# NVlabs/ODISE

Hardware: NVIDIA H100
Metric: images/sec @1024x1024 panoptic inference (ODISE hot path) (higher is better)
Workload: dtype f16q8

## Files before the change

include/odise_b200.h:

```cpp
#ifndef ODISE_B200_H_
#define ODISE_B200_H_

#include <stdint.h>

#ifdef __cplusplus
extern "C" {
#endif

#define ODISE_OK 0
#define ODISE_ERR_ARG 10001
#define ODISE_ERR_ALIGN 10002
#define ODISE_ERR_DRIVER 10003
#define ODISE_ERR_TENSORMAP 10004
#define ODISE_ERR_WORKSPACE 10005
#define ODISE_ERR_UNSUPPORTED 10006

#define ODISE_ACT_NONE 0
#define ODISE_ACT_RELU 1
#define ODISE_ACT_SILU 2
#define ODISE_ACT_GELU 3
#define ODISE_ACT_QUICKGELU 4

#define ODISE_PLANES_BF16 0
#define ODISE_PLANES_F16 1
// ... 96 lines not shown
int odise_msda_fused_box_backward_det_f16(const void* value, const int64_t* spatial_shapes, const int64_t* level_start,
                                          const float* ref, const void* offs, const void* logits, const void* grad_out,
                                          void* grad_value, void* grad_offs, void* grad_logits,
                                          int N, int S, int M, int D, int L, int Lq, int P, void* workspace,
                                          void* stream);
int odise_msda_fused_box_backward_det_bf16(const void* value, const int64_t* spatial_shapes,
                                           const int64_t* level_start, const float* ref, const void* offs,
                                           const void* logits, const void* grad_out, void* grad_value,
                                           void* grad_offs, void* grad_logits, int N, int S, int M, int D, int L,
                                           int Lq, int P, void* workspace, void* stream);

typedef struct odise_gemm_desc {
  int M, N, K, batch;
  int nmma;
  int conv3x3;
  int conv_C, conv_H, conv_W;
  const void* a_hi; const void* a_lo; long long lda; long long a_batch_stride;
  const void* b_hi; const void* b_lo; long long ldb; long long b_batch_stride;
  float alpha;
  const float* bias;
  const float* rowbias; int rows_per_group; long long rowbias_ld;
  int act;
  const float* residual; long long ld_residual; long long residual_batch_stride;
  float* out_f32; long long ld_out; long long out_batch_stride;
  void* out_hi; void* out_lo; long long ld_out_bf16; long long out_bf16_batch_stride;
  int split_k; void* workspace; long long workspace_bytes;
  int force_bn;
  const float* bias_m;
  int conv_mode;
  int geglu;
  float* gn_partial;
  long long gn_seg_stride; long long gn_plane_stride;
  int out_planes_fp16;
} odise_gemm_desc;
int odise_gemm_bf16(const odise_gemm_desc* desc, void* stream);
int odise_gemm_tile_policy(int M, int N, int K, int batch, int conv3x3, int nmma, int* bn, int* pair);
int odise_profile_begin(void);
int odise_profile_end(long long* launches, double* total_ms, double* total_flops);


int odise_split_f32(const float* x, long long ldx, void* hi, void* lo, long long ldo, long long rows, int cols,
                    void* stream);
int odise_split_f16_f32(const float* x, long long ldx, void* hi, void* lo, long long ldo, long long rows, int cols,
                        void* stream);
int odise_groupnorm_stats_f32(const float* x, long long ldx, float* mean, float* rstd, int B, int HW, int C, int G,
                              float eps, void* stream);
int odise_groupnorm_stats_bs_f32(const float* x, long long ldx, long long x_bs, float* mean, float* rstd, int B,
                                 int HW, int C, int G, float eps, void* stream);
long long odise_groupnorm_ws_floats(int B, int HW, int C, int G);
int odise_groupnorm_stats_ws_f32(const float* x, long long ldx, long long x_bs, float* ws, float* mean, float* rstd,
                                 int B, int HW, int C, int G, float eps, void* stream);
int odise_groupnorm_finalize_seg_f32(const float* partial, long long seg_stride, long long plane_stride, float* mean,
                                     float* rstd, int B, int HW, int C, int G, float eps, void* stream);
int odise_groupnorm_apply_f32(const float* x, long long ldx, const float* mean, const float* rstd,
                              const float* gamma, const float* beta, int act, float* y, long long ldy, void* hi,
                              void* lo, long long ldo, int B, int HW, int C, int G, void* stream);
int odise_groupnorm_apply_bs_f32(const float* x, long long ldx, long long x_bs, const float* mean, const float* rstd,
                                 const float* gamma, const float* beta, int act, float* y, long long ldy,
                                 long long y_bs, void* hi, void* lo, long long ldo, long long o_bs, int B, int HW,
                                 int C, int G, void* stream);
int odise_groupnorm_apply_res_f32(const float* x, long long ldx, const float* mean, const float* rstd,
                                  const float* gamma, const float* beta, const float* res, long long ldres, int act,
                                  float* y, long long ldy, int accumulate, void* hi, void* lo, long long ldo, int B,
                                  int HW, int C, int G, void* stream);
int odise_bcast_fma_f32(const float* a0, const float* ta, const float* p, float* out, int B, int T, int C,
                        void* stream);
// ... 126 lines not shown
```

odise_b200/csrc/gemm_tc.cu:

```cuda
#include "ptx.cuh"
#include "wgmma.cuh"
#include "odise_b200.h"
#include "launch_count.h"
#include <cudaTypedefs.h>
#include <mutex>
#include <map>
#include <cstring>
#include <vector>
#include <cstdlib>
#include <cstdio>

namespace ob {

struct GemmParams {
  int M, N, K, batch;
  int a_batched, b_batched;
  int conv, C, H, W, bw, bh, bb;
  int nseg;
  int cstride, cpad;
  int tiles_m, tiles_n, splits, kblocks;
  float alpha;
  const float* bias;
  const float* bias_m;
  const float* rowbias;
// ... 144 lines not shown
      for (int t = 0; t < 4; ++t)
        split_f16(acc[t], *reinterpret_cast<uint16_t*>(&h[t]), *reinterpret_cast<uint16_t*>(&l[t]));
      if (vec) {
        *reinterpret_cast<uint2*>(dh) = *reinterpret_cast<const uint2*>(h);
        if (dl) *reinterpret_cast<uint2*>(dl) = *reinterpret_cast<const uint2*>(l);
      } else {
#pragma unroll
        for (int j = 0; j < 4; ++j) if (j < valid) { dh[j] = h[j]; if (dl) dl[j] = l[j]; }
      }
    } else if (vec) {
      store_planes<4>(dh, dl, acc);
    } else {
#pragma unroll
      for (int j = 0; j < 4; ++j) if (j < valid) store_planes<1>(dh + j, dl ? dl + j : nullptr, acc + j);
    }
  }
}

template <int BN, int NMMA>
struct GemmCfg {
  static constexpr int BM = 128, BK = 64;
  static constexpr int A_BYTES = BM * BK * 2;
  static constexpr int B_BYTES = BN * BK * 2;
  static constexpr int PLANES = (NMMA == 1) ? 1 : 2;
  static constexpr int STAGE_BYTES = PLANES * (A_BYTES + B_BYTES);
  static constexpr int THREADS = 384;
  static constexpr int EPI_BYTES = 8 * 32 * 16 * 4;
  static constexpr int STAGES_RAW = (232448 - EPI_BYTES - 256 - 1024) / STAGE_BYTES;
  static constexpr int STAGES = STAGES_RAW > 8 ? 8 : STAGES_RAW;
  static constexpr int SMEM_BYTES = STAGES * STAGE_BYTES + EPI_BYTES + 256 + 1024;
  static_assert(STAGES >= 2, "GEMM tile does not fit shared memory");
};

template <int BN, int NMMA, int EPI>
__global__ void __launch_bounds__(GemmCfg<BN, NMMA>::THREADS, 1)
gemm_tc_kernel(const __grid_constant__ CUtensorMap tmAh, const __grid_constant__ CUtensorMap tmAl,
               const __grid_constant__ CUtensorMap tmBh, const __grid_constant__ CUtensorMap tmBl, const GemmParams p) {
  using Cfg = GemmCfg<BN, NMMA>;
  extern __shared__ uint8_t smem_raw[];
  uint8_t* smem = reinterpret_cast<uint8_t*>((reinterpret_cast<uintptr_t>(smem_raw) + 1023) & ~uintptr_t(1023));
  float* epi_smem = reinterpret_cast<float*>(smem + Cfg::STAGES * Cfg::STAGE_BYTES);
  uint64_t* bars = reinterpret_cast<uint64_t*>(smem + Cfg::STAGES * Cfg::STAGE_BYTES + Cfg::EPI_BYTES);
  uint64_t* full = bars;
  uint64_t* empty = bars + Cfg::STAGES;

  const int warp = threadIdx.x >> 5;
  const int lane = threadIdx.x & 31;

  if (warp == 8 && lane == 0) {
    tma_prefetch_desc(&tmAh);
    tma_prefetch_desc(&tmBh);
    if (NMMA != 1) {
      tma_prefetch_desc(&tmAl);
      tma_prefetch_desc(&tmBl);
    }
    for (int s = 0; s < Cfg::STAGES; ++s) {
      mbar_init(&full[s], 1);
      mbar_init(&empty[s], 8);
    }
    fence_barrier_init();
  }
  __syncthreads();

  const int tiles_per_z = p.tiles_m * p.tiles_n * p.splits;
  const int total_tiles = tiles_per_z * p.batch;
  const int kb_per_split = (p.kblocks + p.splits - 1) / p.splits;

  if (warp >= 8) {
    setmaxnreg_dec<40>();
    if (warp == 8 && lane == 0) {
      int stage = 0;
      uint32_t phase = 0;
      const int cpk = p.conv ? (p.C / 64) : 1;
      for (int tile = blockIdx.x; tile < total_tiles; tile += gridDim.x) {
        const int z = tile / tiles_per_z;
        int r = tile - z * tiles_per_z;
        const int sp = r / (p.tiles_m * p.tiles_n);
        r -= sp * (p.tiles_m * p.tiles_n);
        const int mt = r / p.tiles_n, nt = r % p.tiles_n;
        const int m0 = mt * 128, n0 = nt * BN;
        const int kb0 = sp * kb_per_split;
        const int kb1 = min(p.kblocks, kb0 + kb_per_split);
        int b0 = 0, h0 = 0, w0 = 0;
        if (p.conv) {
          const int hw = p.H * p.W;
          b0 = m0 / hw;
          const int rem = m0 - b0 * hw;
          h0 = rem / p.W;
          w0 = rem - h0 * p.W;
        }
        for (int kb = kb0; kb < kb1; ++kb) {
          mbar_wait(&empty[stage], phase ^ 1);
          uint8_t* st = smem + stage * Cfg::STAGE_BYTES;
          mbar_arrive_expect_tx(&full[stage], Cfg::STAGE_BYTES);
          if (p.conv) {
            const int tap = kb / cpk, cc = kb - tap * cpk;
            const int kh = tap / 3, kw = tap - kh * 3;
            if (p.nseg == 1) {
              const int cx = w0 * p.cstride + kw - p.cpad, cy = h0 * p.cstride + kh - p.cpad;
              tma_load_4d(st, &tmAh, &full[stage], cc * 64, cx, cy, b0);
              if (NMMA != 1) tma_load_4d(st + Cfg::A_BYTES, &tmAl, &full[stage], cc * 64, cx, cy, b0);
            } else {
              const int hw = p.H * p.W;
              for (int sg = 0; sg < p.nseg; ++sg) {
                const int m = m0 + sg * p.bw;
                const int bi = m / hw, rem = m - bi * hw;
                const int hi_ = rem / p.W, wi = rem - hi_ * p.W;
                const int cx = wi * p.cstride + kw - p.cpad, cy = hi_ * p.cstride + kh - p.cpad;
                uint8_t* sa = st + sg * p.bw * 128;
                tma_load_4d(sa, &tmAh, &full[stage], cc * 64, cx, cy, bi);
                if (NMMA != 1) tma_load_4d(sa + Cfg::A_BYTES, &tmAl, &full[stage], cc * 64, cx, cy, bi);
              }
            }
          } else {
            const int za = p.a_batched ? z : 0;
            tma_load_3d(st, &tmAh, &full[stage], kb * 64, m0, za);
            if (NMMA != 1) tma_load_3d(st + Cfg::A_BYTES, &tmAl, &full[stage], kb * 64, m0, za);
          }
          const int zb = p.b_batched ? z : 0;
          uint8_t* sb = st + Cfg::PLANES * Cfg::A_BYTES;
          tma_load_3d(sb, &tmBh, &full[stage], kb * 64, n0, zb);
          if (NMMA != 1) tma_load_3d(sb + Cfg::B_BYTES, &tmBl, &full[stage], kb * 64, n0, zb);
          if (++stage == Cfg::STAGES) { stage = 0; phase ^= 1; }
        }
      }
    }
    return;
  }

  setmaxnreg_inc<232>();
  const int wg = warp >> 2, wi = warp & 3;
  int stage = 0;
  uint32_t phase = 0;
  float acc[BN / 2];
  float acc2[BN / 2];
  float* stg_wg = epi_smem + wg * (4 * 512);
  float* stg = stg_wg + wi * 512;
  const int cq = lane & 3, rsub = lane >> 2;
  for (int tile = blockIdx.x; tile < total_tiles; tile += gridDim.x) {
    const int z = tile / tiles_per_z;
    int r = tile - z * tiles_per_z;
    const int sp = r / (p.tiles_m * p.tiles_n);
    r -= sp * (p.tiles_m * p.tiles_n);
    const int mt = r / p.tiles_n, nt = r % p.tiles_n;
    const int n0 = nt * BN;
    const int kb0 = sp * kb_per_split;
    const int kb1 = min(p.kblocks, kb0 + kb_per_split);

    if (kb0 >= kb1) {
#pragma unroll
      for (int i = 0; i < BN / 2; ++i) acc[i] = 0.f;
      if constexpr (NMMA == 2) {
#pragma unroll
        for (int i = 0; i < BN / 2; ++i) acc2[i] = 0.f;
      }
    }
    int prev = -1;
    for (int kb = kb0; kb < kb1; ++kb) {
      mbar_wait(&full[stage], phase);
      const uint32_t sa = smem_u32(smem + stage * Cfg::STAGE_BYTES) + wg * (64 * 128);
      const uint32_t sb = smem_u32(smem + stage * Cfg::STAGE_BYTES + Cfg::PLANES * Cfg::A_BYTES);
      reg_fence(acc);
      if constexpr (NMMA == 2) reg_fence(acc2);
      wgmma_fence();
#pragma unroll
      for (int k = 0; k < 4; ++k) {
        const uint64_t a_hi = wgmma_desc_sw128(sa + k * 32);
        const uint64_t b_hi = wgmma_desc_sw128(sb + k * 32);
        const int accum = (kb > kb0 || k > 0) ? 1 : 0;
        if constexpr (NMMA == 2) wgmma_f16(acc, a_hi, b_hi, accum);
        else wgmma_bf16(acc, a_hi, b_hi, accum);
        if constexpr (NMMA == 3) {
          wgmma_bf16(acc, a_hi, wgmma_desc_sw128(sb + Cfg::B_BYTES + k * 32), 1);
          wgmma_bf16(acc, wgmma_desc_sw128(sa + Cfg::A_BYTES + k * 32), b_hi, 1);
        }
      }
      if constexpr (NMMA == 2) {
        const uint32_t a2 = sa + Cfg::A_BYTES, b2 = sb + Cfg::B_BYTES;
#pragma unroll
        for (int k = 0; k < 2; ++k) {
          wgmma_e5m2(acc2, wgmma_desc_sw128(a2 + k * 32), wgmma_desc_sw128(b2 + 64 + k * 32), (kb > kb0 || k > 0) ? 1 : 0);
          wgmma_e5m2(acc2, wgmma_desc_sw128(a2 + 64 + k * 32), wgmma_desc_sw128(b2 + k * 32), 1);
        }
      }
      wgmma_commit();
      wgmma_wait<1>();
      if (prev >= 0 && lane == 0) mbar_arrive(&empty[prev]);
      prev = stage;
      if (++stage == Cfg::STAGES) { stage = 0; phase ^= 1; }
    }
    wgmma_wait<0>();
    reg_fence(acc);
    if (prev >= 0 && lane == 0) mbar_arrive(&empty[prev]);
    if constexpr (NMMA == 2) {
      reg_fence(acc2);
#pragma unroll
      for (int i = 0; i < BN / 2; ++i) acc[i] += acc2[i];
    }

    const int m_base = mt * 128 + wg * 64 + (wi & 1) * 32;
    const bool interior = p.vec_ok && p.splits == 1 && (mt * 128 + 128 <= p.M) && (n0 + BN <= p.N);
    constexpr bool EXTRA = EPI == 1, GEGLU = EPI == 2;
    const bool has_bias = p.bias != nullptr, has_res = EXTRA && p.res != nullptr;
    const bool to_f32 = p.D != nullptr, to_hi = p.Dh != nullptr, to_lo = p.Dl != nullptr;
    const int act = p.act;
    const float alpha = p.alpha;
    const bool has_gn = !GEGLU && p.gnp != nullptr;
    const long long gn_seg = ((long long)z * p.M + m_base) >> 5;
#pragma unroll 1
    for (int ch = 0; ch < BN / 32; ++ch) {
      named_bar_sync(1 + wg, 128);
#pragma unroll
      for (int j = 0; j < BN / 8; ++j) {
        if ((j >> 2) != ch) continue;
#pragma unroll
        for (int h = 0; h < 2; ++h) {
          const int rw = wi * 16 + rsub + 8 * h, cc = 8 * (j & 3) + 2 * cq;
          const int rr = rw & 31, c16 = cc & 15;
          float* dst = stg_wg + ((rw >> 5) | ((cc >> 4) << 1)) * 512 + rr * 16 + (((c16 >> 2) ^ ((rr >> 1) & 3)) << 2) + (c16 & 3);
          *reinterpret_cast<float2*>(dst) = make_float2(acc[4 * j + 2 * h], acc[4 * j + 2 * h + 1]);
        }
      }
      named_bar_sync(1 + wg, 128);
      const int c0 = ch * 32 + (wi >> 1) * 16;
      if (interior) {
        GnAcc gacc;
// ... 126 lines not shown
    for (int sp = 0; sp < p.splits; ++sp) {
      const float* src = p.partial + ((long long)(sp * p.batch + z) * p.M + m) * p.N + n;
#pragma unroll
      for (int j = 0; j < 4; ++j) if (j < valid) acc[j] += src[j];
    }
    epilogue_quad(p, z, m, n, valid, make_float4(acc[0], acc[1], acc[2], acc[3]));
  }
}

static PFN_cuTensorMapEncodeTiled_v12000 get_encode() {
  static PFN_cuTensorMapEncodeTiled_v12000 fn = nullptr;
  static std::once_flag once;
  std::call_once(once, [] {
    void* f = nullptr;
    cudaDriverEntryPointQueryResult q;
    if (cudaGetDriverEntryPoint("cuTensorMapEncodeTiled", &f, cudaEnableDefault, &q) == cudaSuccess &&
        q == cudaDriverEntryPointSuccess)
      fn = reinterpret_cast<PFN_cuTensorMapEncodeTiled_v12000>(f);
  });
  return fn;
}

static int encode_map(CUtensorMap* tm, const void* base, int rank, const cuuint64_t* dims,
                      const cuuint64_t* strides_bytes, const cuuint32_t* box, int spatial_stride = 1) {
  auto enc = get_encode();
  if (!enc) return ODISE_ERR_DRIVER;
  cuuint32_t estr[5] = {1, (cuuint32_t)spatial_stride, (cuuint32_t)spatial_stride, 1, 1};
  CUresult r = enc(tm, CU_TENSOR_MAP_DATA_TYPE_BFLOAT16, rank, const_cast<void*>(base), dims, strides_bytes, box,
                   estr, CU_TENSOR_MAP_INTERLEAVE_NONE, CU_TENSOR_MAP_SWIZZLE_128B,
                   CU_TENSOR_MAP_L2_PROMOTION_L2_256B, CU_TENSOR_MAP_FLOAT_OOB_FILL_NONE);
  return r == CUDA_SUCCESS ? ODISE_OK : ODISE_ERR_TENSORMAP;
}

struct ProfRec { cudaEvent_t a, b; double flops; int M, N, K, batch, conv, bn, nmma, splits; };
static std::vector<ProfRec> g_prof;
static bool g_prof_on = false;

int num_sms() {
  static int n = 0;
  if (!n) {
    int dev = 0;
    cudaGetDevice(&dev);
    cudaDeviceGetAttribute(&n, cudaDevAttrMultiProcessorCount, dev);
    if (n <= 0) n = 132;
  }
  return n;
}

template <int BN, int NMMA, int EPI>
static int launch_cfg(const CUtensorMap& ah, const CUtensorMap& al, const CUtensorMap& bh, const CUtensorMap& bl,
                      const GemmParams& p, cudaStream_t stream) {
  using Cfg = GemmCfg<BN, NMMA>;
  static bool attr_set = false;
  if (!attr_set) {
    cudaError_t e = cudaFuncSetAttribute(gemm_tc_kernel<BN, NMMA, EPI>, cudaFuncAttributeMaxDynamicSharedMemorySize,
                                         Cfg::SMEM_BYTES);
    if (e != cudaSuccess) return (int)e;
    attr_set = true;
  }
  const int total = p.tiles_m * p.tiles_n * p.splits * p.batch;
  const int grid = total < num_sms() ? total : num_sms();
  gemm_tc_kernel<BN, NMMA, EPI><<<grid, Cfg::THREADS, Cfg::SMEM_BYTES, stream>>>(ah, al, bh, bl, p);
  return (int)cudaGetLastError();
}

static int pick_tile(int M, int N, int K, int batch, int forced, bool conv, int nmma) {
  const int cands[4] = {256, 160, 128, 64};
  const double eff[4] = {0.833, 0.933, 1.0, 1.333};
  const double epi_k = 480.0;
  const long long tm = (M + 127) / 128;
  double best = 1e30;
  int c = 128;
  for (int i = 0; i < 4; ++i) {
    const int bn = cands[i];
    if (forced && bn != forced) continue;
    if (nmma == 2 && bn > 128) continue;
    const long long tn = (N + bn - 1) / bn;
    const long long units = tm * tn * batch;
    const long long waves = (units + num_sms() - 1) / num_sms();
    double cost;
    if (conv) {
      cost = (double)waves * bn * eff[i] + 0.02 * bn;
    } else {
      const double mma = (double)bn * K * eff[i], epi = (double)bn * epi_k;
      cost = (double)waves * ((mma > epi ? mma : epi) + 20000.0);
    }
    if (cost < best) { best = cost; c = bn; }
  }
  return c;
}

}

using namespace ob;

// ... 90 lines not shown
    if (d->lda % 8 || d->a_batch_stride % 8) return ODISE_ERR_ALIGN;
    const long long bs = d->a_batch_stride ? d->a_batch_stride : (long long)d->M * d->lda;
    cuuint64_t dims[3] = {(cuuint64_t)d->K, (cuuint64_t)d->M, (cuuint64_t)(d->a_batch_stride ? d->batch : 1)};
    cuuint64_t str[2] = {(cuuint64_t)d->lda * 2, (cuuint64_t)bs * 2};
    cuuint32_t box[3] = {64, 128, 1};
    rc = encode_map(&ah, d->a_hi, 3, dims, str, box);
    if (rc) return rc;
    if (d->nmma == 2) {
      dims[0] = (cuuint64_t)((d->K + 63) / 64 * 64);
      if ((long long)dims[0] > d->lda) return ODISE_ERR_ALIGN;
    }
    rc = encode_map(&al, d->nmma != 1 ? d->a_lo : d->a_hi, 3, dims, str, box);
    if (rc) return rc;
  }
  p.tiles_m = (d->M + 127) / 128;
  if (d->ldb % 8 || d->b_batch_stride % 8) return ODISE_ERR_ALIGN;
  if (d->nmma == 2 && (long long)((d->K + 63) / 64 * 64) > d->ldb) return ODISE_ERR_ALIGN;
  if (d->geglu) {
    if (!d->out_hi || d->out_f32 || d->residual || d->rowbias || d->bias_m || d->split_k > 1 || d->N % 16 ||
        !p.vec_ok || d->act != ODISE_ACT_NONE)
      return ODISE_ERR_UNSUPPORTED;
  }
  p.kblocks = (d->K + 63) / 64;
  p.splits = d->split_k > 1 ? d->split_k : 1;
  if (p.splits > p.kblocks) p.splits = p.kblocks;
  if (p.splits > 1) {
    if (!d->workspace ||
        d->workspace_bytes < (long long)p.splits * d->batch * d->M * d->N * (long long)sizeof(float))
      return ODISE_ERR_WORKSPACE;
    p.partial = reinterpret_cast<float*>(d->workspace);
  }
  const int epi = d->geglu ? 2 : ((d->residual || d->rowbias || d->bias_m) ? 1 : 0);

  auto launch_with = [&](int bn) -> int {
    p.tiles_n = (d->N + bn - 1) / bn;
    const long long bs = d->b_batch_stride ? d->b_batch_stride : (long long)d->N * d->ldb;
    cuuint64_t dims[3] = {(cuuint64_t)d->K, (cuuint64_t)d->N, (cuuint64_t)(d->b_batch_stride ? d->batch : 1)};
    cuuint64_t str[2] = {(cuuint64_t)d->ldb * 2, (cuuint64_t)bs * 2};
    cuuint32_t box[3] = {64, (cuuint32_t)bn, 1};
    int r = encode_map(&bh, d->b_hi, 3, dims, str, box);
    if (r) return r;
    if (d->nmma == 2) dims[0] = (cuuint64_t)((d->K + 63) / 64 * 64);
    r = encode_map(&bl, d->nmma != 1 ? d->b_lo : d->b_hi, 3, dims, str, box);
    if (r) return r;
#define ODISE_LAUNCH(BN_, NM_)                                                   \
  r = epi == 2   ? launch_cfg<BN_, NM_, 2>(ah, al, bh, bl, p, stream)            \
      : epi == 1 ? launch_cfg<BN_, NM_, 1>(ah, al, bh, bl, p, stream)            \
                 : launch_cfg<BN_, NM_, 0>(ah, al, bh, bl, p, stream)
    if (d->nmma == 3) {
      switch (bn) {
        case 64: ODISE_LAUNCH(64, 3); break;
        case 128: ODISE_LAUNCH(128, 3); break;
        case 160: ODISE_LAUNCH(160, 3); break;
        default: ODISE_LAUNCH(256, 3); break;
      }
    } else if (d->nmma == 2) {
      if (bn == 64) ODISE_LAUNCH(64, 2);
      else ODISE_LAUNCH(128, 2);
    } else {
      switch (bn) {
        case 64: ODISE_LAUNCH(64, 1); break;
        case 128: ODISE_LAUNCH(128, 1); break;
        case 160: ODISE_LAUNCH(160, 1); break;
        default: ODISE_LAUNCH(256, 1); break;
      }
    }
#undef ODISE_LAUNCH
    if (r) return r;
    if (p.splits > 1) {
      const long long total = (long long)p.batch * p.M * ((p.N + 3) / 4);
      int blocks = (int)((total + 127) / 128);
      if (blocks > num_sms() * 8) blocks = num_sms() * 8;
      gemm_splitk_reduce_kernel<<<blocks, 128, 0, stream>>>(p);
      r = (int)cudaGetLastError();
    }
    return r;
  };

  int BN;
  {
    static const bool tune = !(getenv("ODISE_GEMM_AUTOTUNE") && atoi(getenv("ODISE_GEMM_AUTOTUNE")) == 0);
    const int fbn = (d->force_bn == 64 || d->force_bn == 128 || d->force_bn == 160 || d->force_bn == 256) ? d->force_bn : 0;
    BN = pick_tile(d->M, d->N, d->K, d->batch, fbn, d->conv3x3 != 0, d->nmma);
    struct Key {
      int v[13];
      bool operator<(const Key& o) const { return memcmp(v, o.v, sizeof(v)) < 0; }
    };
    static std::map<Key, int> cache;
    static std::mutex mu;
    const Key key{{d->M, d->N, d->K, d->batch, d->conv3x3 ? 1 + d->conv_mode : 0, d->conv_W, d->nmma, epi, p.splits,
                  (d->out_f32 ? 1 : 0) | (d->out_hi ? 2 : 0) | (d->out_planes_fp16 << 2), p.gnp ? 1 : 0, d->act, p.vec_ok}};
    cudaStreamCaptureStatus cap = cudaStreamCaptureStatusNone;
    cudaStreamIsCapturing(stream, &cap);
    std::lock_guard<std::mutex> lk(mu);
    auto it = cache.find(key);
    if (it != cache.end()) {
      BN = it->second;
    } else if (tune && !fbn && !g_prof_on && cap == cudaStreamCaptureStatusNone &&
               !(d->residual && (const void*)d->residual == (const void*)d->out_f32)) {
      const int cands[4] = {256, 160, 128, 64};
      cudaEvent_t e0, e1;
      cudaEventCreate(&e0);
      cudaEventCreate(&e1);
      float best = 1e30f;
      int bc = BN;
      for (int i = 0; i < 4; ++i) {
        const int c = cands[i];
        if (c == 64 && d->N > 96 && (long long)p.tiles_m * ((d->N + 127) / 128) * d->batch >= 2 * num_sms()) continue;
        if (c > 128 && (d->N <= 64 || d->nmma == 2)) continue;
        if (launch_with(c)) { (void)cudaGetLastError(); continue; }
        cudaEventRecord(e0, stream);
        int r2 = launch_with(c);
        if (!r2) r2 = launch_with(c);
        cudaEventRecord(e1, stream);
        if (r2 || cudaEventSynchronize(e1) != cudaSuccess) { (void)cudaGetLastError(); continue; }
        float ms = 0.f;
        cudaEventElapsedTime(&ms, e0, e1);
        if (ms < best) { best = ms; bc = c; }
      }
      cudaEventDestroy(e0);
      cudaEventDestroy(e1);
      cache[key] = bc;
      BN = bc;
      if (getenv("ODISE_VERBOSE"))
        fprintf(stderr, "odise_b200: gemm %d x %d x %d (batch %d, conv %d, nmma %d, epi %d): BN %d, %.1f us\n", d->M, d->N,
                d->K, d->batch, d->conv3x3, d->nmma, epi, BN, best * 500.f);
    }
  }

  ProfRec rec{};
  if (g_prof_on) {
    cudaEventCreate(&rec.a);
    cudaEventCreate(&rec.b);
    rec.flops = 2.0 * d->M * d->N * (double)d->K * d->batch;
    rec.M = d->M; rec.N = d->N; rec.K = d->K; rec.batch = d->batch; rec.conv = d->conv3x3; rec.bn = BN;
    rec.nmma = d->nmma; rec.splits = p.splits;
    cudaEventRecord(rec.a, stream);
  }
  rc = launch_with(BN);
  if (rc) return rc;
  count_launch(p.splits > 1 ? 2 : 1);
  if (g_prof_on) {
    cudaEventRecord(rec.b, stream);
    g_prof.push_back(rec);
  }
  return rc;
}

extern "C" int odise_gemm_tile_policy(int M, int N, int K, int batch, int conv3x3, int nmma, int* bn, int* pair) {
  if (M <= 0 || N <= 0 || K <= 0 || batch <= 0 || !bn || !pair || nmma < 1 || nmma > 3) return ODISE_ERR_ARG;
  *bn = pick_tile(M, N, K, batch, 0, conv3x3 != 0, nmma);
  *pair = 0;
  return ODISE_OK;
}

extern "C" int odise_profile_begin(void) {
  for (auto& r : g_prof) { cudaEventDestroy(r.a); cudaEventDestroy(r.b); }
  g_prof.clear();
  g_prof_on = true;
  return ODISE_OK;
}

extern "C" int odise_profile_end(long long* launches, double* total_ms, double* total_flops) {
  g_prof_on = false;
  cudaError_t e = cudaDeviceSynchronize();
  if (e != cudaSuccess) return (int)e;
  double ms = 0, fl = 0;
  FILE* fcsv = nullptr;
  if (const char* path = getenv("ODISE_PROFILE_CSV")) fcsv = fopen(path, "a");
  if (fcsv) fprintf(fcsv, "M,N,K,batch,conv,bn,nmma,splits,ms,tflops\n");
  for (auto& r : g_prof) {
    float t = 0;
    cudaEventElapsedTime(&t, r.a, r.b);
    ms += t;
    fl += r.flops;
    if (fcsv)
      fprintf(fcsv, "%d,%d,%d,%d,%d,%d,%d,%d,%.4f,%.1f\n", r.M, r.N, r.K, r.batch, r.conv, r.bn, r.nmma, r.splits, t,
              r.flops / (t * 1e9));
  }
  if (fcsv) fclose(fcsv);
  if (launches) *launches = (long long)g_prof.size();
  if (total_ms) *total_ms = ms;
  if (total_flops) *total_flops = fl;
  for (auto& r : g_prof) { cudaEventDestroy(r.a); cudaEventDestroy(r.b); }
  g_prof.clear();
  return ODISE_OK;
}
```

odise_b200/csrc/ptx.cuh:

```cuda
#pragma once
#include <cuda.h>
#include <cuda_runtime.h>
#include <cuda_bf16.h>
#include <cuda_fp16.h>
#include <cuda_fp8.h>
#include <stdint.h>
#include <stdio.h>

namespace ob {

__device__ __forceinline__ uint32_t smem_u32(const void* p) {
  return static_cast<uint32_t>(__cvta_generic_to_shared(p));
}
__device__ __forceinline__ uint32_t lane_id() { return threadIdx.x & 31; }

__device__ __forceinline__ bool elect_one() {
  uint32_t pred = 0;
  asm volatile(
      "{\n\t.reg .pred P;\n\telect.sync _|P, 0xffffffff;\n\tselp.u32 %0, 1, 0, P;\n\t}\n"
      : "=r"(pred));
  return pred != 0;
}

__device__ __forceinline__ void mbar_init(uint64_t* bar, uint32_t count) {
  asm volatile("mbarrier.init.shared::cta.b64 [%0], %1;" ::"r"(smem_u32(bar)), "r"(count) : "memory");
}
__device__ __forceinline__ void fence_barrier_init() {
  asm volatile("fence.mbarrier_init.release.cluster;" ::: "memory");
}
__device__ __forceinline__ void mbar_arrive_expect_tx(uint64_t* bar, uint32_t bytes) {
  asm volatile("mbarrier.arrive.expect_tx.shared::cta.b64 _, [%0], %1;" ::"r"(smem_u32(bar)), "r"(bytes)
               : "memory");
}
__device__ __forceinline__ void mbar_arrive(uint64_t* bar) {
  asm volatile("mbarrier.arrive.shared::cta.b64 _, [%0];" ::"r"(smem_u32(bar)) : "memory");
}
__device__ __forceinline__ bool mbar_try_wait(uint64_t* bar, uint32_t parity) {
  uint32_t ok;
  asm volatile(
      "{\n\t.reg .pred P;\n\t"
      "mbarrier.try_wait.parity.shared::cta.b64 P, [%1], %2;\n\t"
      "selp.u32 %0, 1, 0, P;\n\t}\n"
      : "=r"(ok)
      : "r"(smem_u32(bar)), "r"(parity)
      : "memory");
  return ok != 0;
}
__device__ __forceinline__ void mbar_wait(uint64_t* bar, uint32_t parity) {
  if (mbar_try_wait(bar, parity)) return;
  long long t0 = clock64();
  while (!mbar_try_wait(bar, parity)) {
    if (clock64() - t0 > 4000000000LL) __trap();
  }
}
template <int R>
__device__ __forceinline__ void setmaxnreg_dec() {
  asm volatile("setmaxnreg.dec.sync.aligned.u32 %0;" ::"n"(R));
}
template <int R>
__device__ __forceinline__ void setmaxnreg_inc() {
  asm volatile("setmaxnreg.inc.sync.aligned.u32 %0;" ::"n"(R));
}

__device__ __forceinline__ void tma_prefetch_desc(const CUtensorMap* m) {
  asm volatile("prefetch.tensormap [%0];" ::"l"(reinterpret_cast<uint64_t>(m)) : "memory");
}
__device__ __forceinline__ void tma_load_3d(void* smem_dst, const CUtensorMap* m, uint64_t* bar, int c0, int c1,
                                            int c2) {
  asm volatile(
      "cp.async.bulk.tensor.3d.shared::cluster.global.mbarrier::complete_tx::bytes [%0], [%1, {%3, %4, %5}], [%2];"
      ::"r"(smem_u32(smem_dst)), "l"(reinterpret_cast<uint64_t>(m)), "r"(smem_u32(bar)), "r"(c0), "r"(c1), "r"(c2)
      : "memory");
}
__device__ __forceinline__ void tma_load_4d(void* smem_dst, const CUtensorMap* m, uint64_t* bar, int c0, int c1,
                                            int c2, int c3) {
  asm volatile(
      "cp.async.bulk.tensor.4d.shared::cluster.global.mbarrier::complete_tx::bytes [%0], [%1, {%3, %4, %5, %6}], "
      "[%2];" ::"r"(smem_u32(smem_dst)),
      "l"(reinterpret_cast<uint64_t>(m)), "r"(smem_u32(bar)), "r"(c0), "r"(c1), "r"(c2), "r"(c3)
      : "memory");
}

__device__ __forceinline__ void named_bar_sync(uint32_t id, uint32_t threads) {
  asm volatile("bar.sync %0, %1;" ::"r"(id), "r"(threads) : "memory");
}
__device__ __forceinline__ void wgmma_fence() { asm volatile("wgmma.fence.sync.aligned;" ::: "memory"); }
__device__ __forceinline__ void wgmma_commit() { asm volatile("wgmma.commit_group.sync.aligned;" ::: "memory"); }
template <int N>
__device__ __forceinline__ void wgmma_wait() {
  asm volatile("wgmma.wait_group.sync.aligned %0;" ::"n"(N) : "memory");
}
template <int R>
__device__ __forceinline__ void reg_fence(float (&d)[R]) {
#pragma unroll
  for (int i = 0; i < R; ++i) asm volatile("" : "+f"(d[i])::"memory");
}

__device__ __forceinline__ uint64_t wgmma_desc_sw128(uint32_t smem_addr) {
  uint64_t d = 0;
  d |= static_cast<uint64_t>((smem_addr & 0x3FFFF) >> 4);
  d |= static_cast<uint64_t>(1) << 16;
  d |= static_cast<uint64_t>(1024 >> 4) << 32;
  d |= static_cast<uint64_t>(1) << 62;
  return d;
// ... 103 lines not shown
```

odise_b200/lib.py:

```python
import ctypes
import os
from ctypes import c_int, c_float, c_longlong, c_void_p, POINTER

import torch

_HERE = os.path.dirname(os.path.abspath(__file__))
_LIB_PATH = os.path.join(_HERE, "libodise_b200.so")

ACT_NONE, ACT_RELU, ACT_SILU, ACT_GELU, ACT_QUICKGELU = 0, 1, 2, 3, 4


class OdiseError(RuntimeError):
    pass


class GemmDesc(ctypes.Structure):
    _fields_ = [
        ("M", c_int), ("N", c_int), ("K", c_int), ("batch", c_int),
        ("nmma", c_int), ("conv3x3", c_int),
        ("conv_C", c_int), ("conv_H", c_int), ("conv_W", c_int),
        ("a_hi", c_void_p), ("a_lo", c_void_p), ("lda", c_longlong), ("a_batch_stride", c_longlong),
        ("b_hi", c_void_p), ("b_lo", c_void_p), ("ldb", c_longlong), ("b_batch_stride", c_longlong),
        ("alpha", c_float),
        ("bias", c_void_p),
        ("rowbias", c_void_p), ("rows_per_group", c_int), ("rowbias_ld", c_longlong),
        ("act", c_int),
        ("residual", c_void_p), ("ld_residual", c_longlong), ("residual_batch_stride", c_longlong),
        ("out_f32", c_void_p), ("ld_out", c_longlong), ("out_batch_stride", c_longlong),
        ("out_hi", c_void_p), ("out_lo", c_void_p), ("ld_out_bf16", c_longlong), ("out_bf16_batch_stride", c_longlong),
        ("split_k", c_int), ("workspace", c_void_p), ("workspace_bytes", c_longlong),
        ("force_bn", c_int),
        ("bias_m", c_void_p),
        ("conv_mode", c_int),
        ("geglu", c_int),
        ("gn_partial", c_void_p), ("gn_seg_stride", c_longlong), ("gn_plane_stride", c_longlong),
        ("out_planes_fp16", c_int),
    ]


_lib = None

_SIGS = {
    "odise_msda_forward_f32": [c_void_p] * 6 + [c_int] * 7 + [c_void_p],
    "odise_msda_fused_f32": [c_void_p] * 9 + [c_int] * 7 + [c_void_p],
    "odise_msda_forward_f64": [c_void_p] * 6 + [c_int] * 7 + [c_void_p],
    "odise_msda_backward_f32": [c_void_p] * 9 + [c_int] * 7 + [c_void_p],
    "odise_msda_backward_f64": [c_void_p] * 9 + [c_int] * 7 + [c_void_p],
    "odise_msda_fused_backward_f32": [c_void_p] * 10 + [c_int] * 7 + [c_void_p],
    "odise_msda_fused_f16": [c_void_p] * 7 + [c_int] * 7 + [c_void_p],
    "odise_msda_fused_bf16": [c_void_p] * 7 + [c_int] * 7 + [c_void_p],
    "odise_msda_fused_backward_f16": [c_void_p] * 10 + [c_int] * 7 + [c_void_p],
    "odise_msda_fused_backward_bf16": [c_void_p] * 10 + [c_int] * 7 + [c_void_p],
    "odise_msda_det_workspace_bytes": [c_int] * 4,
    "odise_msda_backward_det_f32": [c_void_p] * 9 + [c_int] * 7 + [c_void_p, c_void_p],
    "odise_msda_backward_det_f64": [c_void_p] * 9 + [c_int] * 7 + [c_void_p, c_void_p],
    "odise_msda_fused_backward_det_f32": [c_void_p] * 10 + [c_int] * 7 + [c_void_p, c_void_p],
    "odise_msda_fused_backward_det_f16": [c_void_p] * 10 + [c_int] * 7 + [c_void_p, c_void_p],
    "odise_msda_fused_backward_det_bf16": [c_void_p] * 10 + [c_int] * 7 + [c_void_p, c_void_p],
    "odise_msda_fused_box_f32": [c_void_p] * 7 + [c_int] * 7 + [c_void_p],
    "odise_msda_fused_box_f16": [c_void_p] * 7 + [c_int] * 7 + [c_void_p],
    "odise_msda_fused_box_bf16": [c_void_p] * 7 + [c_int] * 7 + [c_void_p],
    "odise_msda_fused_box_backward_f32": [c_void_p] * 10 + [c_int] * 7 + [c_void_p],
    "odise_msda_fused_box_backward_f16": [c_void_p] * 10 + [c_int] * 7 + [c_void_p],
    "odise_msda_fused_box_backward_bf16": [c_void_p] * 10 + [c_int] * 7 + [c_void_p],
    "odise_msda_fused_box_backward_det_f32": [c_void_p] * 10 + [c_int] * 7 + [c_void_p, c_void_p],
    "odise_msda_fused_box_backward_det_f16": [c_void_p] * 10 + [c_int] * 7 + [c_void_p, c_void_p],
    "odise_msda_fused_box_backward_det_bf16": [c_void_p] * 10 + [c_int] * 7 + [c_void_p, c_void_p],
    "odise_masked_xattn_workspace_bytes": [c_int] * 4,
    "odise_masked_xattn_forward_f32": [c_void_p] * 4 + [c_longlong] + [c_void_p] * 2 + [c_int] * 5 + [c_void_p] * 2,
# ... 275 lines not shown
def auto_split(M, N, K, batch=1, sms=132):
    tm = (M + 127) // 128
    kblocks = (K + 63) // 64
    unit = 0.68 / (64 * 128)
    best = (None, 1e30)
    for bn in (128, 160, 256):
        tiles = tm * ((N + bn - 1) // bn) * batch
        for s in (1, 2, 3, 4):
            if s > 1 and kblocks // s < 16:
                continue
            waves = (tiles * s + sms - 1) // sms
            cost = waves * (K / s) * bn * unit
            if s > 1:
                cost += 6.0 + 8.0 * s * M * N * batch / 5.0e6
            if cost < best[1]:
                best = ((bn, s), cost)
    bn, s = best[0]
    return (bn, s) if s > 1 else (0, 1)


def conv_ok(H, W):
    import math
    if W % 128 == 0:
        return True
    if 128 % W == 0:
        bh = min(128 // W, H)
        if H % bh == 0 and 128 % (W * bh) == 0:
            return True
    return math.gcd(W, 128) % 8 == 0


def gemm(a, b, *, M=None, N=None, K=None, nmma=3, batch=1, a_bs=0, b_bs=0, conv=None, alpha=1.0, bias=None, bias_m=None,
         rowbias=None, rows_per_group=1, act=ACT_NONE, residual=None, ld_res=None, res_bs=0, out=None, ld_out=None,
         out_bs=0, out_planes=None, outp_bs=0, split_k=1, workspace=None, force_bn=0, geglu=False, conv_mode=0, gn=None):
    d = GemmDesc()
    d.M = M if M is not None else a.rows
    d.N = N if N is not None else b.rows
    d.K = K if K is not None else (9 * conv[0] if conv else a.cols)
    d.batch = batch
    if conv:
        d.conv3x3, d.conv_C, d.conv_H, d.conv_W = 1, conv[0], conv[1], conv[2]
    if a.f16 or b.f16:
        raise OdiseError("gemm: fp16 planes are attention-kernel operands (V^T), not GEMM inputs")
    if a.fmt != b.fmt:
        raise OdiseError(f"gemm: operand formats differ ({a.fmt} x {b.fmt})")
    if a.fmt == "q8":
        if nmma == 1:
            raise OdiseError("gemm: F16Q8 operands have no plain-bf16 mode")
        nmma = 2
    elif nmma == 2:
        nmma = 3
    d.nmma = nmma
    d.a_hi, d.a_lo, d.lda, d.a_batch_stride = _ptr(a.hi), _ptr(a.lo), a.ld, a_bs
    d.b_hi, d.b_lo, d.ldb, d.b_batch_stride = _ptr(b.hi), _ptr(b.lo), b.ld, b_bs
    d.alpha = alpha
    d.bias = _ptr(bias)
    d.bias_m = _ptr(bias_m)
    if rowbias is not None:
        d.rowbias, d.rows_per_group, d.rowbias_ld = _ptr(rowbias), rows_per_group, rowbias.stride(0)
    d.act = act
    if residual is not None:
        d.residual = _ptr(residual)
        d.ld_residual = ld_res if ld_res is not None else residual.stride(-2)
        d.residual_batch_stride = res_bs
    if out is not None:
        d.out_f32 = _ptr(out)
        d.ld_out = ld_out if ld_out is not None else out.stride(-2)
        d.out_batch_stride = out_bs
    if out_planes is not None:
        d.out_hi, d.out_lo, d.ld_out_bf16 = _ptr(out_planes.hi), _ptr(out_planes.lo), out_planes.ld
        d.out_bf16_batch_stride = outp_bs
        d.out_planes_fp16 = out_planes.code
    d.split_k = split_k
    if split_k > 1:
        need = split_k * batch * d.M * d.N * 4
        if workspace is None or workspace.numel() * workspace.element_size() < need:
            raise OdiseError("gemm: split_k needs a workspace of %d bytes" % need)
        d.workspace, d.workspace_bytes = _ptr(workspace), workspace.numel() * workspace.element_size()
    d.force_bn = force_bn
    if gn is not None:
        if split_k > 1 or gn.missing or d.M % 32 or gn.C != d.N or gn.rows != d.M * batch:
            gn.missing = True
        else:
            d.gn_partial = gn.ptr
            d.gn_seg_stride, d.gn_plane_stride = 3 * gn.Ctot, gn.Ctot
    d.geglu = 1 if geglu else 0
    d.conv_mode = conv_mode
    _check(load().odise_gemm_bf16(ctypes.byref(d), _stream()), "odise_gemm_bf16")
    return out if out is not None else out_planes


def gemm_tile_policy(M, N, K, batch=1, conv=False, nmma=2):
    bn, pair = c_int(0), c_int(0)
    _check(load().odise_gemm_tile_policy(M, N, K, batch, 1 if conv else 0, nmma, ctypes.byref(bn), ctypes.byref(pair)),
           "odise_gemm_tile_policy")
    return bn.value, bool(pair.value)


def msda_forward(value, spatial_shapes, level_start_index, sampling_locations, attention_weights, im2col_step=128):
    for t, nm in ((value, "value"), (sampling_locations, "sampling_loc"), (attention_weights, "attn_weight")):
        if not t.is_cuda:
            raise OdiseError(f"{nm} must be a CUDA tensor")
        if not t.is_contiguous():
            raise OdiseError(f"{nm} tensor has to be contiguous")
        _req(t, torch.float32, nm)
    N, S, M, D = value.shape
    _, Lq, _, L, P, _ = sampling_locations.shape
    step = min(N, im2col_step)
    if N % step != 0:
        raise OdiseError(f"batch({N}) must divide im2col_step({step})")
    ss = spatial_shapes.to(device=value.device, dtype=torch.int64).contiguous()
    ls = level_start_index.to(device=value.device, dtype=torch.int64).contiguous()
# ... 291 lines not shown
```

Baseline: 12.34.

## Add thread-block-cluster TMA multicast of B tiles to the GEMM kernel

```diff
diff --git a/include/odise_b200.h b/include/odise_b200.h
--- a/include/odise_b200.h
+++ b/include/odise_b200.h
@@ -152,6 +152,7 @@
   float* gn_partial;
   long long gn_seg_stride; long long gn_plane_stride;
   int out_planes_fp16;
+  int force_cluster;
 } odise_gemm_desc;
 int odise_gemm_bf16(const odise_gemm_desc* desc, void* stream);
 int odise_gemm_tile_policy(int M, int N, int K, int batch, int conv3x3, int nmma, int* bn, int* pair);
diff --git a/odise_b200/csrc/gemm_tc.cu b/odise_b200/csrc/gemm_tc.cu
--- a/odise_b200/csrc/gemm_tc.cu
+++ b/odise_b200/csrc/gemm_tc.cu
@@ -200,11 +200,13 @@
   static_assert(STAGES >= 2, "GEMM tile does not fit shared memory");
 };
 
-template <int BN, int NMMA, int EPI>
+template <int BN, int NMMA, int EPI, int CM>
 __global__ void __launch_bounds__(GemmCfg<BN, NMMA>::THREADS, 1)
 gemm_tc_kernel(const __grid_constant__ CUtensorMap tmAh, const __grid_constant__ CUtensorMap tmAl,
                const __grid_constant__ CUtensorMap tmBh, const __grid_constant__ CUtensorMap tmBl, const GemmParams p) {
   using Cfg = GemmCfg<BN, NMMA>;
+  static_assert(CM == 1 || CM == 2 || CM == 4, "cluster size");
+  static_assert((BN / CM) % 8 == 0, "B slices start on whole 1024-byte swizzle atoms");
   extern __shared__ uint8_t smem_raw[];
   uint8_t* smem = reinterpret_cast<uint8_t*>((reinterpret_cast<uintptr_t>(smem_raw) + 1023) & ~uintptr_t(1023));
   float* epi_smem = reinterpret_cast<float*>(smem + Cfg::STAGES * Cfg::STAGE_BYTES);
@@ -224,13 +226,15 @@
     }
     for (int s = 0; s < Cfg::STAGES; ++s) {
       mbar_init(&full[s], 1);
-      mbar_init(&empty[s], 8);
+      mbar_init(&empty[s], 8 * CM);
     }
     fence_barrier_init();
   }
   __syncthreads();
-
-  const int tiles_per_z = p.tiles_m * p.tiles_n * p.splits;
+  if constexpr (CM > 1) cluster_sync();
+
+  const int crank = CM > 1 ? (int)cluster_ctarank() : 0;
+  const int tiles_per_z = (p.tiles_m + CM - 1) / CM * p.tiles_n * p.splits;
   const int total_tiles = tiles_per_z * p.batch;
   const int kb_per_split = (p.kblocks + p.splits - 1) / p.splits;
 
@@ -240,12 +244,12 @@
       int stage = 0;
       uint32_t phase = 0;
       const int cpk = p.conv ? (p.C / 64) : 1;
-      for (int tile = blockIdx.x; tile < total_tiles; tile += gridDim.x) {
+      for (int tile = blockIdx.x / CM; tile < total_tiles; tile += gridDim.x / CM) {
         const int z = tile / tiles_per_z;
         int r = tile - z * tiles_per_z;
-        const int sp = r / (p.tiles_m * p.tiles_n);
-        r -= sp * (p.tiles_m * p.tiles_n);
-        const int mt = r / p.tiles_n, nt = r % p.tiles_n;
+        const int sp = r / ((p.tiles_m + CM - 1) / CM * p.tiles_n);
+        r -= sp * ((p.tiles_m + CM - 1) / CM * p.tiles_n);
+        const int mt = r / p.tiles_n * CM + crank, nt = r % p.tiles_n;
         const int m0 = mt * 128, n0 = nt * BN;
         const int kb0 = sp * kb_per_split;
         const int kb1 = min(p.kblocks, kb0 + kb_per_split);
@@ -287,8 +291,22 @@
           }
           const int zb = p.b_batched ? z : 0;
           uint8_t* sb = st + Cfg::PLANES * Cfg::A_BYTES;
-          tma_load_3d(sb, &tmBh, &full[stage], kb * 64, n0, zb);
-          if (NMMA != 1) tma_load_3d(sb + Cfg::B_BYTES, &tmBl, &full[stage], kb * 64, n0, zb);
+          if constexpr (CM == 1) {
+            tma_load_3d(sb, &tmBh, &full[stage], kb * 64, n0, zb);
+            if (NMMA != 1) tma_load_3d(sb + Cfg::B_BYTES, &tmBl, &full[stage], kb * 64, n0, zb);
+          } else {
+            constexpr int ROWS = BN / CM;
+            constexpr uint16_t ALL = (1u << CM) - 1;
+            uint8_t* sbr = sb + crank * ROWS * 128;
+            tma_load_3d_multicast(sbr, &tmBh, &full[stage], kb * 64, n0 + crank * ROWS, zb, ALL);
+            if (NMMA != 1) tma_load_3d_multicast(sbr + Cfg::B_BYTES, &tmBl, &full[stage], kb * 64, n0 + crank * ROWS, zb, ALL);
+          }
+          if (++stage == Cfg::STAGES) { stage = 0; phase ^= 1; }
+        }
+      }
+      if constexpr (CM > 1) {
+        for (int s = 0; s < Cfg::STAGES; ++s) {
+          mbar_wait(&empty[stage], phase ^ 1);
           if (++stage == Cfg::STAGES) { stage = 0; phase ^= 1; }
         }
       }
@@ -305,12 +323,20 @@
   float* stg_wg = epi_smem + wg * (4 * 512);
   float* stg = stg_wg + wi * 512;
   const int cq = lane & 3, rsub = lane >> 2;
-  for (int tile = blockIdx.x; tile < total_tiles; tile += gridDim.x) {
+  auto release = [&](int s) {
+    if constexpr (CM == 1) {
+      mbar_arrive(&empty[s]);
+    } else {
+#pragma unroll
+      for (int c = 0; c < CM; ++c) mbar_arrive_cluster(&empty[s], c);
+    }
+  };
+  for (int tile = blockIdx.x / CM; tile < total_tiles; tile += gridDim.x / CM) {
     const int z = tile / tiles_per_z;
     int r = tile - z * tiles_per_z;
-    const int sp = r / (p.tiles_m * p.tiles_n);
-    r -= sp * (p.tiles_m * p.tiles_n);
-    const int mt = r / p.tiles_n, nt = r % p.tiles_n;
+    const int sp = r / ((p.tiles_m + CM - 1) / CM * p.tiles_n);
+    r -= sp * ((p.tiles_m + CM - 1) / CM * p.tiles_n);
+    const int mt = r / p.tiles_n * CM + crank, nt = r % p.tiles_n;
     const int n0 = nt * BN;
     const int kb0 = sp * kb_per_split;
     const int kb1 = min(p.kblocks, kb0 + kb_per_split);
@@ -353,13 +379,13 @@
       }
       wgmma_commit();
       wgmma_wait<1>();
-      if (prev >= 0 && lane == 0) mbar_arrive(&empty[prev]);
+      if (prev >= 0 && lane == 0) release(prev);
       prev = stage;
       if (++stage == Cfg::STAGES) { stage = 0; phase ^= 1; }
     }
     wgmma_wait<0>();
     reg_fence(acc);
-    if (prev >= 0 && lane == 0) mbar_arrive(&empty[prev]);
+    if (prev >= 0 && lane == 0) release(prev);
     if constexpr (NMMA == 2) {
       reg_fence(acc2);
 #pragma unroll
@@ -552,7 +578,7 @@
   return r == CUDA_SUCCESS ? ODISE_OK : ODISE_ERR_TENSORMAP;
 }
 
-struct ProfRec { cudaEvent_t a, b; double flops; int M, N, K, batch, conv, bn, nmma, splits; };
+struct ProfRec { cudaEvent_t a, b; double flops; int M, N, K, batch, conv, bn, nmma, splits, cluster; };
 static std::vector<ProfRec> g_prof;
 static bool g_prof_on = false;
 
@@ -567,20 +593,49 @@
   return n;
 }
 
-template <int BN, int NMMA, int EPI>
+template <int BN, int NMMA, int EPI, int CM>
 static int launch_cfg(const CUtensorMap& ah, const CUtensorMap& al, const CUtensorMap& bh, const CUtensorMap& bl,
                       const GemmParams& p, cudaStream_t stream) {
   using Cfg = GemmCfg<BN, NMMA>;
+  auto kern = gemm_tc_kernel<BN, NMMA, EPI, CM>;
+  cudaLaunchAttribute at[1];
+  at[0].id = cudaLaunchAttributeClusterDimension;
+  at[0].val.clusterDim.x = CM; at[0].val.clusterDim.y = 1; at[0].val.clusterDim.z = 1;
   static bool attr_set = false;
+  static int max_clusters = 0;
   if (!attr_set) {
-    cudaError_t e = cudaFuncSetAttribute(gemm_tc_kernel<BN, NMMA, EPI>, cudaFuncAttributeMaxDynamicSharedMemorySize,
-                                         Cfg::SMEM_BYTES);
+    cudaError_t e = cudaFuncSetAttribute(kern, cudaFuncAttributeMaxDynamicSharedMemorySize, Cfg::SMEM_BYTES);
     if (e != cudaSuccess) return (int)e;
+    if constexpr (CM > 1) {
+      cudaLaunchConfig_t q{};
+      q.gridDim = dim3(CM, 1, 1);
+      q.blockDim = dim3(Cfg::THREADS, 1, 1);
+      q.dynamicSmemBytes = Cfg::SMEM_BYTES;
+      q.attrs = at;
+      q.numAttrs = 1;
+      e = cudaOccupancyMaxActiveClusters(&max_clusters, kern, &q);
+      if (e != cudaSuccess) return (int)e;
+      if (max_clusters <= 0) return (int)cudaErrorInvalidConfiguration;
+    }
     attr_set = true;
   }
-  const int total = p.tiles_m * p.tiles_n * p.splits * p.batch;
-  const int grid = total < num_sms() ? total : num_sms();
-  gemm_tc_kernel<BN, NMMA, EPI><<<grid, Cfg::THREADS, Cfg::SMEM_BYTES, stream>>>(ah, al, bh, bl, p);
+  if constexpr (CM == 1) {
+    const int total = p.tiles_m * p.tiles_n * p.splits * p.batch;
+    const int grid = total < num_sms() ? total : num_sms();
+    kern<<<grid, Cfg::THREADS, Cfg::SMEM_BYTES, stream>>>(ah, al, bh, bl, p);
+  } else {
+    if (p.splits != 1) return ODISE_ERR_UNSUPPORTED;
+    const int units = (p.tiles_m + CM - 1) / CM * p.tiles_n * p.batch;
+    cudaLaunchConfig_t c{};
+    c.gridDim = dim3((units < max_clusters ? units : max_clusters) * CM, 1, 1);
+    c.blockDim = dim3(Cfg::THREADS, 1, 1);
+    c.dynamicSmemBytes = Cfg::SMEM_BYTES;
+    c.stream = stream;
+    c.attrs = at;
+    c.numAttrs = 1;
+    const cudaError_t e = cudaLaunchKernelEx(&c, kern, ah, al, bh, bl, p);
+    if (e != cudaSuccess) return (int)e;
+  }
   return (int)cudaGetLastError();
 }
 
@@ -737,21 +792,25 @@
   }
   const int epi = d->geglu ? 2 : ((d->residual || d->rowbias || d->bias_m) ? 1 : 0);
 
-  auto launch_with = [&](int bn) -> int {
+  auto launch_with = [&](int bn, int cm) -> int {
     p.tiles_n = (d->N + bn - 1) / bn;
     const long long bs = d->b_batch_stride ? d->b_batch_stride : (long long)d->N * d->ldb;
     cuuint64_t dims[3] = {(cuuint64_t)d->K, (cuuint64_t)d->N, (cuuint64_t)(d->b_batch_stride ? d->batch : 1)};
     cuuint64_t str[2] = {(cuuint64_t)d->ldb * 2, (cuuint64_t)bs * 2};
-    cuuint32_t box[3] = {64, (cuuint32_t)bn, 1};
+    cuuint32_t box[3] = {64, (cuuint32_t)(bn / cm), 1};
     int r = encode_map(&bh, d->b_hi, 3, dims, str, box);
     if (r) return r;
     if (d->nmma == 2) dims[0] = (cuuint64_t)((d->K + 63) / 64 * 64);
     r = encode_map(&bl, d->nmma != 1 ? d->b_lo : d->b_hi, 3, dims, str, box);
     if (r) return r;
+#define ODISE_LAUNCH_CM(BN_, NM_, CM_)                                           \
+  r = epi == 2   ? launch_cfg<BN_, NM_, 2, CM_>(ah, al, bh, bl, p, stream)       \
+      : epi == 1 ? launch_cfg<BN_, NM_, 1, CM_>(ah, al, bh, bl, p, stream)       \
+                 : launch_cfg<BN_, NM_, 0, CM_>(ah, al, bh, bl, p, stream)
 #define ODISE_LAUNCH(BN_, NM_)                                                   \
-  r = epi == 2   ? launch_cfg<BN_, NM_, 2>(ah, al, bh, bl, p, stream)            \
-      : epi == 1 ? launch_cfg<BN_, NM_, 1>(ah, al, bh, bl, p, stream)            \
-                 : launch_cfg<BN_, NM_, 0>(ah, al, bh, bl, p, stream)
+  if (cm == 4) { ODISE_LAUNCH_CM(BN_, NM_, 4); }                                 \
+  else if (cm == 2) { ODISE_LAUNCH_CM(BN_, NM_, 2); }                            \
+  else { ODISE_LAUNCH_CM(BN_, NM_, 1); }
     if (d->nmma == 3) {
       switch (bn) {
         case 64: ODISE_LAUNCH(64, 3); break;
@@ -760,8 +819,11 @@
         default: ODISE_LAUNCH(256, 3); break;
       }
     } else if (d->nmma == 2) {
-      if (bn == 64) ODISE_LAUNCH(64, 2);
-      else ODISE_LAUNCH(128, 2);
+      if (bn == 64) {
+        ODISE_LAUNCH(64, 2);
+      } else {
+        ODISE_LAUNCH(128, 2);
+      }
     } else {
       switch (bn) {
         case 64: ODISE_LAUNCH(64, 1); break;
@@ -771,6 +833,7 @@
       }
     }
 #undef ODISE_LAUNCH
+#undef ODISE_LAUNCH_CM
     if (r) return r;
     if (p.splits > 1) {
       const long long total = (long long)p.batch * p.M * ((p.N + 3) / 4);
@@ -782,7 +845,9 @@
     return r;
   };
 
-  int BN;
+  if (d->force_cluster != 0 && d->force_cluster != 1 && d->force_cluster != 2 && d->force_cluster != 4) return ODISE_ERR_ARG;
+  if (d->force_cluster > 1 && p.splits > 1) return ODISE_ERR_UNSUPPORTED;
+  int BN, CM = 1;
   {
     static const bool tune = !(getenv("ODISE_GEMM_AUTOTUNE") && atoi(getenv("ODISE_GEMM_AUTOTUNE")) == 0);
     const int fbn = (d->force_bn == 64 || d->force_bn == 128 || d->force_bn == 160 || d->force_bn == 256) ? d->force_bn : 0;
@@ -791,7 +856,7 @@
       int v[13];
       bool operator<(const Key& o) const { return memcmp(v, o.v, sizeof(v)) < 0; }
     };
-    static std::map<Key, int> cache;
+    static std::map<Key, std::pair<int, int>> cache;
     static std::mutex mu;
     const Key key{{d->M, d->N, d->K, d->batch, d->conv3x3 ? 1 + d->conv_mode : 0, d->conv_W, d->nmma, epi, p.splits,
                   (d->out_f32 ? 1 : 0) | (d->out_hi ? 2 : 0) | (d->out_planes_fp16 << 2), p.gnp ? 1 : 0, d->act, p.vec_ok}};
@@ -800,38 +865,45 @@
     std::lock_guard<std::mutex> lk(mu);
     auto it = cache.find(key);
     if (it != cache.end()) {
-      BN = it->second;
-    } else if (tune && !fbn && !g_prof_on && cap == cudaStreamCaptureStatusNone &&
+      BN = it->second.first;
+      CM = it->second.second;
+    } else if (tune && !fbn && !d->force_cluster && !g_prof_on && cap == cudaStreamCaptureStatusNone &&
                !(d->residual && (const void*)d->residual == (const void*)d->out_f32)) {
       const int cands[4] = {256, 160, 128, 64};
+      const int cms = (p.splits == 1 && p.tiles_m >= 2) ? 3 : 1;
       cudaEvent_t e0, e1;
       cudaEventCreate(&e0);
       cudaEventCreate(&e1);
       float best = 1e30f;
-      int bc = BN;
+      int bc = BN, cc = 1;
       for (int i = 0; i < 4; ++i) {
         const int c = cands[i];
         if (c == 64 && d->N > 96 && (long long)p.tiles_m * ((d->N + 127) / 128) * d->batch >= 2 * num_sms()) continue;
         if (c > 128 && (d->N <= 64 || d->nmma == 2)) continue;
-        if (launch_with(c)) { (void)cudaGetLastError(); continue; }
-        cudaEventRecord(e0, stream);
-        int r2 = launch_with(c);
-        if (!r2) r2 = launch_with(c);
-        cudaEventRecord(e1, stream);
-        if (r2 || cudaEventSynchronize(e1) != cudaSuccess) { (void)cudaGetLastError(); continue; }
-        float ms = 0.f;
-        cudaEventElapsedTime(&ms, e0, e1);
-        if (ms < best) { best = ms; bc = c; }
+        for (int j = 0; j < cms; ++j) {
+          const int cm = 1 << j;
+          if (launch_with(c, cm)) { (void)cudaGetLastError(); continue; }
+          cudaEventRecord(e0, stream);
+          int r2 = launch_with(c, cm);
+          if (!r2) r2 = launch_with(c, cm);
+          cudaEventRecord(e1, stream);
+          if (r2 || cudaEventSynchronize(e1) != cudaSuccess) { (void)cudaGetLastError(); continue; }
+          float ms = 0.f;
+          cudaEventElapsedTime(&ms, e0, e1);
+          if (ms < best) { best = ms; bc = c; cc = cm; }
+        }
       }
       cudaEventDestroy(e0);
       cudaEventDestroy(e1);
-      cache[key] = bc;
+      cache[key] = {bc, cc};
       BN = bc;
+      CM = cc;
       if (getenv("ODISE_VERBOSE"))
-        fprintf(stderr, "odise_b200: gemm %d x %d x %d (batch %d, conv %d, nmma %d, epi %d): BN %d, %.1f us\n", d->M, d->N,
-                d->K, d->batch, d->conv3x3, d->nmma, epi, BN, best * 500.f);
-    }
-  }
+        fprintf(stderr, "odise_b200: gemm %d x %d x %d (batch %d, conv %d, nmma %d, epi %d): BN %d, cluster %d, %.1f us\n",
+                d->M, d->N, d->K, d->batch, d->conv3x3, d->nmma, epi, BN, CM, best * 500.f);
+    }
+  }
+  if (d->force_cluster) CM = d->force_cluster;
 
   ProfRec rec{};
   if (g_prof_on) {
@@ -839,10 +911,10 @@
     cudaEventCreate(&rec.b);
     rec.flops = 2.0 * d->M * d->N * (double)d->K * d->batch;
     rec.M = d->M; rec.N = d->N; rec.K = d->K; rec.batch = d->batch; rec.conv = d->conv3x3; rec.bn = BN;
-    rec.nmma = d->nmma; rec.splits = p.splits;
+    rec.nmma = d->nmma; rec.splits = p.splits; rec.cluster = CM;
     cudaEventRecord(rec.a, stream);
   }
-  rc = launch_with(BN);
+  rc = launch_with(BN, CM);
   if (rc) return rc;
   count_launch(p.splits > 1 ? 2 : 1);
   if (g_prof_on) {
@@ -873,15 +945,15 @@
   double ms = 0, fl = 0;
   FILE* fcsv = nullptr;
   if (const char* path = getenv("ODISE_PROFILE_CSV")) fcsv = fopen(path, "a");
-  if (fcsv) fprintf(fcsv, "M,N,K,batch,conv,bn,nmma,splits,ms,tflops\n");
+  if (fcsv) fprintf(fcsv, "M,N,K,batch,conv,bn,nmma,splits,ms,tflops,cluster\n");
   for (auto& r : g_prof) {
     float t = 0;
     cudaEventElapsedTime(&t, r.a, r.b);
     ms += t;
     fl += r.flops;
     if (fcsv)
-      fprintf(fcsv, "%d,%d,%d,%d,%d,%d,%d,%d,%.4f,%.1f\n", r.M, r.N, r.K, r.batch, r.conv, r.bn, r.nmma, r.splits, t,
-              r.flops / (t * 1e9));
+      fprintf(fcsv, "%d,%d,%d,%d,%d,%d,%d,%d,%.4f,%.1f,%d\n", r.M, r.N, r.K, r.batch, r.conv, r.bn, r.nmma, r.splits, t,
+              r.flops / (t * 1e9), r.cluster);
   }
   if (fcsv) fclose(fcsv);
   if (launches) *launches = (long long)g_prof.size();
diff --git a/odise_b200/csrc/ptx.cuh b/odise_b200/csrc/ptx.cuh
--- a/odise_b200/csrc/ptx.cuh
+++ b/odise_b200/csrc/ptx.cuh
@@ -35,6 +35,23 @@
 __device__ __forceinline__ void mbar_arrive(uint64_t* bar) {
   asm volatile("mbarrier.arrive.shared::cta.b64 _, [%0];" ::"r"(smem_u32(bar)) : "memory");
 }
+__device__ __forceinline__ void mbar_arrive_cluster(uint64_t* bar, uint32_t rank) {
+  asm volatile(
+      "{\n\t.reg .b32 ra;\n\t"
+      "mapa.shared::cluster.u32 ra, %0, %1;\n\t"
+      "mbarrier.arrive.shared::cluster.b64 _, [ra];\n\t}\n" ::"r"(smem_u32(bar)), "r"(rank)
+      : "memory");
+}
+
+__device__ __forceinline__ uint32_t cluster_ctarank() {
+  uint32_t r;
+  asm volatile("mov.u32 %0, %%cluster_ctarank;" : "=r"(r));
+  return r;
+}
+__device__ __forceinline__ void cluster_sync() {
+  asm volatile("barrier.cluster.arrive.release;\n\tbarrier.cluster.wait.acquire;" ::: "memory");
+}
+
 __device__ __forceinline__ bool mbar_try_wait(uint64_t* bar, uint32_t parity) {
   uint32_t ok;
   asm volatile(
@@ -70,6 +87,15 @@
   asm volatile(
       "cp.async.bulk.tensor.3d.shared::cluster.global.mbarrier::complete_tx::bytes [%0], [%1, {%3, %4, %5}], [%2];"
       ::"r"(smem_u32(smem_dst)), "l"(reinterpret_cast<uint64_t>(m)), "r"(smem_u32(bar)), "r"(c0), "r"(c1), "r"(c2)
+      : "memory");
+}
+__device__ __forceinline__ void tma_load_3d_multicast(void* smem_dst, const CUtensorMap* m, uint64_t* bar, int c0, int c1,
+                                                      int c2, uint16_t cta_mask) {
+  asm volatile(
+      "cp.async.bulk.tensor.3d.shared::cluster.global.mbarrier::complete_tx::bytes.multicast::cluster"
+      " [%0], [%1, {%3, %4, %5}], [%2], %6;"
+      ::"r"(smem_u32(smem_dst)), "l"(reinterpret_cast<uint64_t>(m)), "r"(smem_u32(bar)), "r"(c0), "r"(c1), "r"(c2),
+      "h"(cta_mask)
       : "memory");
 }
 __device__ __forceinline__ void tma_load_4d(void* smem_dst, const CUtensorMap* m, uint64_t* bar, int c0, int c1,
diff --git a/odise_b200/lib.py b/odise_b200/lib.py
--- a/odise_b200/lib.py
+++ b/odise_b200/lib.py
@@ -35,6 +35,7 @@
         ("geglu", c_int),
         ("gn_partial", c_void_p), ("gn_seg_stride", c_longlong), ("gn_plane_stride", c_longlong),
         ("out_planes_fp16", c_int),
+        ("force_cluster", c_int),
     ]
 
 
@@ -376,7 +377,8 @@
 
 def gemm(a, b, *, M=None, N=None, K=None, nmma=3, batch=1, a_bs=0, b_bs=0, conv=None, alpha=1.0, bias=None, bias_m=None,
          rowbias=None, rows_per_group=1, act=ACT_NONE, residual=None, ld_res=None, res_bs=0, out=None, ld_out=None,
-         out_bs=0, out_planes=None, outp_bs=0, split_k=1, workspace=None, force_bn=0, geglu=False, conv_mode=0, gn=None):
+         out_bs=0, out_planes=None, outp_bs=0, split_k=1, workspace=None, force_bn=0, geglu=False, conv_mode=0, gn=None,
+         force_cluster=0):
     d = GemmDesc()
     d.M = M if M is not None else a.rows
     d.N = N if N is not None else b.rows
@@ -422,6 +424,7 @@
             raise OdiseError("gemm: split_k needs a workspace of %d bytes" % need)
         d.workspace, d.workspace_bytes = _ptr(workspace), workspace.numel() * workspace.element_size()
     d.force_bn = force_bn
+    d.force_cluster = force_cluster
     if gn is not None:
         if split_k > 1 or gn.missing or d.M % 32 or gn.C != d.N or gn.rows != d.M * batch:
             gn.missing = True
```

New measurement: 12.40, median of 6. No clear change (+0.5%).
